# achiever04/face-recognition-platform

Measured on AMD Instinct MI355X. Metric: faces/sec (detect+embed+match) on 1080p @ 100k gallery, higher is better.
Workload: dtype f16; 1 GPU; 32x1080x1920 BGR frames per GPU per step resident in HBM, host results out every step, 2 batches in flight per GPU (one handle = one stream each, used round-robin), forced K=10 faces/frame, 100000-identity fp16 gallery, FRPDet detector fp16 + ArcFace IResNet-100 fp16 (synthetic seeded weights); batch_frames=32, faces_per_frame=10, gallery=100000, streams=1, lanes=2, lane_warmup_steps=20

## Files before the change

### face-recognition-platform_amd/csrc/frp_api.cpp

```cpp
#include <hip/hip_runtime.h>

#include <algorithm>
#include <cmath>
#include <cstdio>
#include <cstdlib>
#include <cstring>
#include <mutex>
#include <string>
#include <vector>

#include "frp.h"
#include "frp_blob.h"
#include "frp_internal.h"
#include "frp_handle.h"

using namespace frp;

#define FRP_WINO_MIN_FACES 128
Switches frp::read_switches() {
    auto set = [](const char* n) { return getenv(n) ? 1 : 0; };
    const char *sm = getenv("FRP_SMALL_M"), *wm = getenv("FRP_WINO_MIN_FACES");
    Switches s{};
    s.small_m = !sm ? 0 : (sm[0] == '0' ? -1 : 1);
    s.wino_min_faces = wm ? atoi(wm) : FRP_WINO_MIN_FACES;
    s.s2 = set("FRP_S2"); s.host_count = set("FRP_HOST_COUNT"); s.match_v1 = set("FRP_MATCH_V1");
    s.no_fused_stem12 = set("FRP_NO_FUSED_STEM12"); s.no_fused_stem = set("FRP_NO_FUSED_STEM");
    s.no_emb_stem = set("FRP_NO_EMB_STEM"); s.no_stem_fuse = set("FRP_NO_STEM_FUSE");
    s.no_wino = set("FRP_NO_WINO"); s.no_kconcat = set("FRP_NO_KCONCAT");
    return s;
}

const ProcessSwitches& frp::process_switches() {
    static const ProcessSwitches s = [] {
        const char* jh = getenv("FRP_JPEG_DEVICE_HUFFMAN");
        const char* js = getenv("FRP_JPEG_SELFSYNC");
        return ProcessSwitches{getenv("FRP_NO_GRAPH") != nullptr, getenv("FRP_C64_ALL") != nullptr, !jh ? 0 : (jh[0] == '0' ? -1 : 1), js && js[0] != '0'};
    }();
    return s;
}

namespace {

float logit_threshold(float t) {
// ... 783 lines not shown
```

### face-recognition-platform_amd/csrc/frp_internal.h

```cpp
#pragma once
#include <hip/hip_runtime.h>
#include <stdint.h>
#include <type_traits>

#define FRP_ACT_NONE 0
#define FRP_ACT_RELU 1
#define FRP_ACT_PRELU 2
#define FRP_FLAG_BORDER_BIAS 1
#define FRP_FLAG_OUT_F32 2
#define FRP_FLAG_RES_UP2 4
#define FRP_FLAG_FLATTEN 8
#define FRP_FLAG_F8 32
#define FRP_FLAG_OUT_FP8 64
#define FRP_CHIP_PIX (112 * 112)
#ifndef FRP_MAX_FACES_CAP
#define FRP_MAX_FACES_CAP 128
#endif

#include "jpeg_host.h"
#include "jpeg_selfsync.h"

namespace frp {

struct Switches {
    int small_m;
    int s2;
    int no_fused_stem12;
    int no_fused_stem;
    int no_emb_stem;
    int no_stem_fuse;
    int wino_min_faces;
    int host_count;
    int match_v1;
    int no_wino;
    int no_kconcat;
};
static_assert(std::has_unique_object_representations_v<Switches>, "run_net keys captured graphs by the bytes of a Switches");
Switches read_switches();

struct ProcessSwitches {
    bool no_graph;
    bool c64_all;
    int jpeg_device_huffman;
    bool jpeg_selfsync;
};
const ProcessSwitches& process_switches();

struct ConvParams {
    const _Float16* x;
    const _Float16* w;
// ... 70 lines not shown
    C64Plan c64;
};
hipError_t conv_derive(ConvParams& p, int* ncu);
ConvRoute conv_pick(const ConvParams& p, int ncu);
hipError_t launch_conv(const ConvParams& p, hipStream_t stream);
hipError_t launch_conv_generic(const ConvParams& p, bool few, hipStream_t stream);
bool conv3x3_rows_eligible(const ConvParams& p);
long conv3x3_lean_default_tiles(const ConvParams& p);
#ifdef FRP_LAB
hipError_t launch_conv3x3_rows(const ConvParams& p, bool few, hipStream_t stream);
#endif
hipError_t launch_conv3x3_lean(const ConvParams& p, bool few, hipStream_t stream);
bool conv3x3_c64_eligible(const ConvParams& p, C64Plan* plan);
bool conv3x3_c64_fuses_stem(int N, int H, int W, int n_cu);
hipError_t launch_conv3x3_c64(const ConvParams& p, const C64Plan& plan, hipStream_t stream);
bool conv3x3_s2_eligible(const ConvParams& p);
hipError_t launch_conv3x3_s2(const ConvParams& p, hipStream_t stream);
int conv3x3_wino_form(const ConvParams& p);
bool conv3x3_wino_shape_ok(int W, int Cin, int ksize, int stride);
bool conv3x3_wino_call_ok(int N, int H, int W, int Cin, int Cout, int ksize, int stride, int n_cu, bool has_res, int dbg);
bool conv3x3_wino_wide_pays(int N, int H, int W, int Cin, int Cout, int n_cu, bool has_res);
#ifdef FRP_LAB
bool conv3x3_wino_lab_shape_ok(int W, int Cin, int ksize, int stride);
#endif
size_t conv3x3_wino_image_bytes(int Cin, int Cout);
hipError_t launch_conv3x3_wino(const ConvParams& p, int form, hipStream_t stream);

hipError_t launch_preprocess(const uint8_t* bgr, int B, int H, int W, long row_stride, long frame_stride,
                             _Float16* out, int Hc, int Wc, int rgb_in, hipStream_t stream);

// ... 272 lines not shown
```

### face-recognition-platform_amd/csrc/kernel_api.cpp

```cpp
#include <hip/hip_runtime.h>

#include <cmath>

#include "frp.h"
#ifdef FRP_LAB
#include "frp_lab.h"
#endif
#include "frp_handle.h"

using namespace frp;

#ifdef FRP_LAB
namespace {
template <typename Launch>
hipError_t time_launches(frp_handle* h, int warm, int iters, Launch launch, float* ms) {
    hipError_t e = hipSuccess;
    for (int i = 0; i < warm && e == hipSuccess; ++i) e = launch();
    if (e == hipSuccess) e = hipEventRecord(h->ev[0], h->stream);
    for (int i = 0; i < iters && e == hipSuccess; ++i) e = launch();
    if (e == hipSuccess) e = hipEventRecord(h->ev[1], h->stream);
    if (e == hipSuccess) e = hipStreamSynchronize(h->stream);
    if (e == hipSuccess) e = hipEventElapsedTime(ms, h->ev[0], h->ev[1]);
    return e;
}
// ... 103 lines not shown
        p.out2 = out2_f8 ? dout2->p : nullptr;
        p.wscale = (const float*)dws->p;
        p.in_scale = in_scale; p.out_scale = out_scale;
        p.N = N; p.H = H; p.W = W; p.Cin = Cin; p.Cout = Cout; p.KS = 3; p.stride = 1; p.act = act;
        p.flags = (flags & (FRP_FLAG_BORDER_BIAS | FRP_FLAG_OUT_FP8)) | FRP_FLAG_F8;
        e = launch_conv(p, h->stream);
    }
    if (e == hipSuccess) e = hipMemcpyAsync(out, dout->p, on * (out8 ? 1 : 2), hipMemcpyDeviceToHost, h->stream);
    if (e == hipSuccess && out2_f8) e = hipMemcpyAsync(out2_f8, dout2->p, on, hipMemcpyDeviceToHost, h->stream);
    hipError_t e2 = hipStreamSynchronize(h->stream);
    if (e != hipSuccess) return fail(h, e == hipErrorInvalidValue ? FRP_ERR_INVALID : FRP_ERR_HIP, std::string("conv2d_f8: ") + hipGetErrorString(e));
    if (e2 != hipSuccess) return fail(h, FRP_ERR_HIP, std::string("conv2d_f8 sync: ") + hipGetErrorString(e2));
    return FRP_OK;
}

int frp_debug_pyramid_merge(frp_handle* h, int32_t n_scales, const int32_t* det_hw, int32_t B, int32_t per_scale, int32_t frame_h,
                            int32_t frame_w, const float* boxes, const float* kps, const float* scores, const int32_t* counts,
                            int32_t max_faces, float nms_iou, float* out_boxes, float* out_kps, float* out_scores, int32_t* out_counts) {
    if (!h) return FRP_ERR_INVALID;
    Guard g(h);
    if (!det_hw || !boxes || !kps || !scores || !counts || !out_boxes || !out_kps || !out_scores || !out_counts)
        return fail(h, FRP_ERR_INVALID, "pyramid_merge: null argument");
    if (n_scales < 1 || n_scales > FRP_PYRAMID_MAX_SCALES || per_scale < 1 || per_scale > FRP_MAX_FACES_CAP ||
        n_scales * per_scale > FRP_PYRAMID_MAX_CAND || max_faces < 1 || max_faces > FRP_MAX_FACES_CAP || B < 1 || B > 1024 || frame_h < 1 ||
        frame_w < 1)
        return fail(h, FRP_ERR_INVALID, "pyramid_merge: 1..4 scales, per_scale and max_faces in 1..128, at most 512 candidates per frame");
    const int S = n_scales, P = per_scale, K = max_faces;
    PyramidMergeParams mp{};
    for (int s = 0; s < S; ++s) {
        mp.det_h[s] = det_hw[2 * s]; mp.det_w[s] = det_hw[2 * s + 1];
// ... 76 lines not shown
        if (with_res) p.out2 = nullptr;
    }
    conv_route_from_abi_flags(flags, p);
    const bool wino_shape = conv3x3_wino_call_ok(N, H, W, Cin, Cout, ksize, stride, h->n_cu, with_res != 0, p.dbg);
    if ((flags & (1 << 16)) && wino_shape) {
        const size_t ib = conv3x3_wino_image_bytes(Cin, Cout);
        if (ensure(h, dwino, ib) == FRP_OK) {
            e = launch_fill_random_f16((_Float16*)dwino->p, (long)(ib / 2), 5u, 1.0f / sqrtf((float)(9 * Cin)), h->stream);
            p.wino_w = (const _Float16*)dwino->p;
        }
    }
    if (stamps_out && ensure(h, dst, 256 * 8 * 8) == FRP_OK) {
        (void)hipMemsetAsync(dst->p, 0, 256 * 8 * 8, h->stream);
        p.stamps = (unsigned long long*)dst->p;
    }
    if (e == hipSuccess) e = time_launches(h, 2, iters, [&] { return launch_conv(p, h->stream); }, &ms);
    if (e == hipSuccess && stamps_out && p.stamps) e = hipMemcpy(stamps_out, p.stamps, 256 * 8 * 8, hipMemcpyDeviceToHost);
    (void)hipStreamSynchronize(h->stream);
    if (e != hipSuccess) return fail(h, FRP_ERR_HIP, std::string("conv_bench: ") + hipGetErrorString(e));
    *ms_avg = ms / iters;
    return FRP_OK;
}

int frp_mfma_peak(frp_handle* h, int32_t waves_per_simd, int32_t iters, float* tflops) {
    if (!h) return FRP_ERR_INVALID;
    Guard g(h);
    const int lds_reads = waves_per_simd >> 4;
    if (lds_reads) waves_per_simd &= 15;
    if (!tflops || iters <= 0 || waves_per_simd < 1 || waves_per_simd > 8 || (lds_reads && (waves_per_simd != 2 || lds_reads < 2 || lds_reads > 4)))
        return fail(h, FRP_ERR_INVALID, "bad arguments");
// ... 39 lines not shown
```

### face-recognition-platform_amd/csrc/net_program.cpp

```cpp
#include "net_program.h"

#include <algorithm>
#include <cmath>
#include <cstdio>
#include <cstring>

#include "frp_handle.h"

namespace frp {

static float fp8_e4m3_value(unsigned char c) {
    const int e = (c >> 3) & 0xF, m = c & 7;
    float v;
    if (e == 15 && m == 7) v = 0.f;
    else if (e == 0) v = std::ldexp((float)m / 8.0f, -6);
    else v = std::ldexp(1.0f + (float)m / 8.0f, e - 7);
    return (c & 0x80) ? -v : v;
}

uint16_t f32_to_f16_bits(float f) {
    uint32_t x;
    memcpy(&x, &f, 4);
    const uint32_t sign = (x >> 16) & 0x8000u;
    x &= 0x7fffffffu;
// ... 234 lines not shown
    if (nb < 0) return;
    const frp_conv_op& b = net.ops[nb];
    const bool plain = !(b.flags & ~FRP_FLAG_BORDER_BIAS) && (b.flags & FRP_FLAG_BORDER_BIAS) && b.out2_buf < 0 && b.res_buf < 0;
    const bool chained = net.kc_src[nb] < 0;
    net.fuse_ok = plain && chained && b.in_buf == a.out_buf && b.out_buf != a.out_buf && b.out_buf != a.in_buf && a.out_buf != a.in_buf &&
                  b.cin == 64 && b.cout == 64 && b.ksize == 3 && b.stride == 1 && b.act == FRP_ACT_PRELU && b.slope_off >= 0;
    net.fuse_even_only = true;
    for (int j = 1; j < (int)net.ops.size(); ++j) {
        const frp_conv_op& o = net.ops[j];
        if (j == nb || (o.in_buf != a.out_buf && o.res_buf != a.out_buf)) continue;
        const bool shortcut = net.kc_skip[j] && o.in_buf == a.out_buf && o.res_buf != a.out_buf && o.ksize == 1 && o.stride == 2;
        if (!shortcut) net.fuse_even_only = false;
    }
}

void analyse_net(Net& net) {
    const int n = (int)net.ops.size();
    net.det_stem = stem_fusable(net);
    net.det_stem12 = stem12_fusable(net);
    net.fc_op = n && (net.ops[n - 1].flags & FRP_FLAG_OUT_F32) ? n - 1 : -1;
    net.next_launch.assign(n, -1);
    for (int i = n - 1, nx = -1; i >= 0; --i) {
        net.next_launch[i] = nx;
        if (!net.kc_skip[i]) nx = i;
    }
    net.emb_stem = net.fuse_ok = net.fuse_even_only = false;
    net.fuse_op = -1;
    if (n) analyse_emb_stem(net);
}

}

int load_program(frp_handle* h, const frp_blob_header& hd, const unsigned char* blob, size_t bytes, const Switches& sw,
                 std::vector<unsigned char>& image) {
    Net &det = h->det, &emb = h->emb;
    det.is_det = true;
    FRPCHK(parse_net(h, blob, bytes, hd.det_ops_offset, hd.n_det_ops, hd.n_det_bufs, hd.det_in_buf, hd.det_in_ch, hd.data_bytes, det));
    FRPCHK(parse_net(h, blob, bytes, hd.emb_ops_offset, hd.n_emb_ops, hd.n_emb_bufs, hd.emb_in_buf, hd.emb_in_ch, hd.data_bytes, emb));
    for (int l = 0; l < 3; ++l)
        if (hd.det_head_buf[l] >= hd.n_det_bufs) return fail(h, FRP_ERR_BLOB, "head buffer id out of range");
    if (hd.emb_out_buf >= hd.n_emb_bufs) return fail(h, FRP_ERR_BLOB, "embedding buffer id out of range");
    image.assign(blob + hd.data_offset, blob + hd.data_offset + hd.data_bytes);
    for (Net* net : {&det, &emb}) {
// ... 1 lines not shown
        net->wino_off.assign(n_ops, -1);
        net->kc_skip.assign(n_ops, 0);
        net->kc_src.assign(n_ops, -1);
        net->kc_w_off.assign(n_ops, -1);
        net->kc_bias_off.assign(n_ops, -1);
        expand_fp8_weights(*net, image);
    }
    if (!sw.no_wino) {
        add_wino_images(emb, FRP_CHIP, [](const frp_conv_op& op, int win) { return conv3x3_wino_shape_ok(win, op.cin, op.ksize, op.stride); }, image);
        add_wino_images(det, 0, [](const frp_conv_op& op, int) { return op.ksize == 3 && op.stride == 1 && !(op.cin & 63) && op.cin >= 128; }, image);
    }
    if (!sw.no_kconcat) {
        plan_kconcat(det, {(int)hd.det_head_buf[0], (int)hd.det_head_buf[1], (int)hd.det_head_buf[2]}, image);
        plan_kconcat(emb, {(int)hd.emb_out_buf}, image);
    }
    analyse_net(det);
    analyse_net(emb);
    return FRP_OK;
}

int plan_net(frp_handle* h, Net& net, int batch, int H, int W, bool skip_input) {
    net.dims.assign(net.n_bufs, TensorDims());
    std::vector<size_t> need(net.n_bufs, 0);
    net.dims[net.in_buf] = {H, W, net.in_ch, false};
    need[net.in_buf] = skip_input ? 0 : (size_t)batch * H * W * net.in_ch * 2;
    for (const frp_conv_op& op : net.ops) {
        if (net.dims[op.in_buf].c == 0) return fail(h, FRP_ERR_BLOB, "program reads an unwritten buffer");
        const TensorDims in = flat_input(net.dims[op.in_buf], op), out = conv_out_dims(in, op);
        if (in.c != op.cin) return fail(h, FRP_ERR_BLOB, "program channel mismatch");
        if (out.h <= 0 || out.w <= 0) return fail(h, FRP_ERR_INVALID, "input too small for the network");
        if (in.f32) return fail(h, FRP_ERR_BLOB, "program reads an fp32 tensor as a conv input");
        const bool op_f8 = (op.flags & FRP_OPFLAG_FP8_MFMA) != 0;
// ... 174 lines not shown
    p.ksplit = ps.n_dev ? -1 : ks;
    p.out = h->splitk_ws.p;
    fc.ksplit = p.ksplit;
    fc.bias = p.bias;
    fc.ktot = op.ksize * op.ksize * op.cin;
}

void charge(const frp_conv_op& op, const TensorDims& out, int batch, PassEffects& fx) {
    const int cin_r = op.real_ch & 0xffff, cout_r = (op.real_ch >> 16) & 0xffff;
    const double fl = 2.0 * batch * out.h * out.w * (double)op.ksize * op.ksize * (cin_r ? cin_r : op.cin) * (cout_r ? cout_r : op.cout);
    fx.flops += fl;
    fx.launches += 1;
    if (op.flags & FRP_OPFLAG_FP8_MFMA) { fx.f8_flops += fl; fx.f8_launches += 1; }
}

int walk(const NetPass& ps, PassEffects& fx) {
    frp_handle* h = ps.h;
    const Net& net = ps.net;
    fx = PassEffects();
    std::vector<TensorDims>& d = fx.dims;
    d.assign(net.n_bufs, TensorDims());
    d[net.in_buf] = {ps.H, ps.W, net.in_ch, false};
    const bool hashing = net.is_det && h->det_hash_on;
    if (hashing) HIPCHK(h, hipMemsetAsync(h->det_hashes.p, 0, 64 * 8, h->stream));
    size_t i = 0;
    FusedStem fused;
    if (ps.stem) FRPCHK(run_det_stems(ps, fx, i));
    else FRPCHK(run_emb_stem(ps, fx, i, fused));
    size_t end = net.ops.size();
    if (net.is_det && h->det_op_limit >= 0) end = std::min(end, (size_t)h->det_op_limit);
    for (; i < end; ++i) {
        const frp_conv_op& op = net.ops[i];
        const TensorDims in = flat_input(d[op.in_buf], op), out = conv_out_dims(in, op);
        if (net.kc_skip[i]) {
            set_out_dims(d, op, out);
            fx.flops += 2.0 * ps.batch * out.h * out.w * (double)op.cin * op.cout;
            continue;
        }
        ConvParams p = conv_params_for(ps, i, in, d, fused);
        if ((int)i == net.fc_op) pick_fc_splitk(ps, op, in, out, p, fx.fc);
        FRPCHK(launched(h, launch_conv(p, h->stream), "launch_conv"));
        set_out_dims(d, op, out);
        if (hashing && i < 64 && !ps.n_dev)
            FRPCHK(launched(h, launch_tensor_hash(net.bufs[op.out_buf].p, (size_t)ps.batch * out.h * out.w * out.c * (out.f32 ? 4 : 2),
                                                  (unsigned long long*)h->det_hashes.p + i, h->stream), "tensor_hash"));
        charge(op, out, ps.batch, fx);
    }
    return FRP_OK;
}

std::string graph_key(const NetPass& ps) {
    char kb[512];
    int len = snprintf(kb, sizeof kb, "%c|%d|%d|%d|%d|%p|%p|", ps.net.is_det ? 'd' : 'e', ps.batch, ps.H, ps.W, (int)ps.allow_wino, (const void*)ps.n_dev,
// ... 95 lines not shown
```

### face-recognition-platform_amd/csrc/net_program.h

```cpp
#pragma once
#include <string>
#include <vector>

#include "frp_blob.h"
#include "frp_internal.h"

struct frp_handle;

namespace frp {

struct DevBuf {
    void* p = nullptr;
    size_t cap = 0;
};

struct TensorDims {
    int h = 0, w = 0, c = 0;
    bool f32 = false;
    bool f8 = false;
};

struct Net {
    std::vector<frp_conv_op> ops;
    int n_bufs = 0;
    int in_buf = 0, in_ch = 0;
    bool is_det = false;
    std::vector<DevBuf> bufs;
    std::vector<TensorDims> dims;
    std::vector<int64_t> wino_off;
    std::vector<int> kc_skip;
    std::vector<int> kc_src;
    std::vector<int64_t> kc_w_off, kc_bias_off;
    bool det_stem = false;
    bool det_stem12 = false;
    bool emb_stem = false;
    int fuse_op = -1;
    bool fuse_ok = false;
    bool fuse_even_only = false;
    int fc_op = -1;
    std::vector<int> next_launch;
};

struct FcSplitK {
    int ksplit = 0, ktot = 0;
    const float* bias = nullptr;
};

struct PassEffects {
    double flops = 0, f8_flops = 0;
    int64_t launches = 0, f8_launches = 0;
    FcSplitK fc;
    std::vector<TensorDims> dims;
};
// ... 24 lines not shown
```

### face-recognition-platform_amd/native.py

```python
from __future__ import annotations

import ctypes as C
import os
import threading
from typing import Optional, Sequence, Tuple

import numpy as np

_HERE = os.path.dirname(os.path.abspath(__file__))
os.environ.setdefault("GPU_MAX_HW_QUEUES", "8")

LIB_PATH = os.environ.get("FRP_LIB") or os.path.join(_HERE, "libfrp.so")

EMB_DIM = 512
CHIP = 112
MAX_FACES_CAP = 128
MAX_TOPK = 64
FLAG_FORCED_K, FLAG_RGB, FLAG_NO_MATCH, FLAG_WITHIN = 1, 2, 4, 8
F32, F16, F64 = 0, 1, 2
JPEG_SUBSAMPLING = {"4:2:0": 420, "4:4:4": 444}
YUV_LAYOUTS = {"NV12": 0, "NV21": 1, "I420": 2, "YV12": 3}
YUV_MATRICES = {"BT601": 0, "BT709": 1, "JFIF": 2}
YUV_DEVICE = 1
QUALITY_TILE_H, QUALITY_TILE_W = 32, 64

ABI_SYMBOLS = [
    "frp_create", "frp_destroy", "frp_last_error", "frp_version", "frp_load_weights",
    "frp_gallery_set", "frp_gallery_set_device", "frp_gallery_reserve", "frp_gallery_commit", "frp_gallery_cancel", "frp_gallery_device_ptr", "frp_gallery_update_row", "frp_gallery_remove_row",
    "frp_jpeg_info_get", "frp_jpeg_coefficients", "frp_upload_jpeg_async", "frp_debug_jpeg_device_batches", "frp_debug_graph_replays",
    "frp_set_jpeg_selfsync", "frp_debug_jpeg_selfsync_batches", "frp_jpeg_selfsync_coefficients",
    "frp_dist_unique_id", "frp_dist_init", "frp_dist_destroy", "frp_gallery_allgather",
    "frp_gallery_size", "frp_gallery_get", "frp_gallery_exact", "frp_gallery_distances", "frp_gallery_get_exact",
    "frp_process_frames", "frp_upload_frames", "frp_process_resident", "frp_fetch_results", "frp_synchronize",
    "frp_host_alloc", "frp_host_free", "frp_upload_frames_async", "frp_swap_frames",
    "frp_upload_yuv", "frp_upload_yuv_async", "frp_get_frames",
    "frp_detect", "frp_detect_resident", "frp_get_det_source", "frp_finish_faces", "frp_process_pyramid", "frp_debug_pyramid_merge", "frp_get_head_map", "frp_debug_det_prefix", "frp_debug_det_hashes", "frp_decode_heads", "frp_align", "frp_debug_align_resident", "frp_embed_aligned", "frp_embed_faces",
    "frp_match", "frp_match_scores", "frp_debug_match_f16", "frp_match_within", "frp_set_within", "frp_fetch_within", "frp_face_quality", "frp_jpeg_encode_headers", "frp_encode_jpeg", "frp_encode_jpeg_coefficients", "frp_conv2d_nhwc", "frp_conv2d_f8", "frp_get_counters", "frp_reset_counters", "frp_set_profile",
]


class FrpConfig(C.Structure):
    _fields_ = [("struct_size", C.c_int32), ("max_batch", C.c_int32), ("max_faces", C.c_int32),
                ("max_h", C.c_int32), ("max_w", C.c_int32), ("profile", C.c_int32), ("reserved", C.c_int32 * 10)]


class FrpCounters(C.Structure):
    _fields_ = [("struct_size", C.c_int32), ("calls", C.c_int32), ("frames", C.c_int64), ("faces", C.c_int64),
                ("ms_h2d", C.c_double), ("ms_preprocess", C.c_double), ("ms_det_conv", C.c_double),
                ("ms_decode", C.c_double), ("ms_align", C.c_double), ("ms_emb_conv", C.c_double),
                ("ms_l2norm", C.c_double), ("ms_match", C.c_double), ("ms_d2h", C.c_double), ("ms_total", C.c_double),
                ("det_conv_flops", C.c_double), ("emb_conv_flops", C.c_double),
                ("det_conv_launches", C.c_int64), ("emb_conv_launches", C.c_int64),
# ... 168 lines not shown
    lib.frp_match_scores.argtypes = [vp, vp, i32, vp, i64]
    if hasattr(lib, "frp_debug_match_f16"):
        lib.frp_debug_match_f16.argtypes = [vp, vp, i32, i32, vp, vp, vp, i64]
    if hasattr(lib, "frp_match_within"):
        lib.frp_match_within.argtypes = [vp, vp, i32, f32, i32, vp, vp, vp]
        lib.frp_set_within.argtypes = [vp, f32, i32]
        lib.frp_fetch_within.argtypes = [vp, i32, i32, i32, vp, vp, vp]
    if hasattr(lib, "frp_face_quality"):
        lib.frp_face_quality.argtypes = [vp, vp, i32, u32, vp]
    if hasattr(lib, "frp_encode_jpeg"):
        lib.frp_jpeg_encode_headers.argtypes = [i32, i32, i32, i32, i32, vp, i64]
        lib.frp_jpeg_encode_headers.restype = i64
        lib.frp_encode_jpeg.argtypes = [vp, vp, i32, i32, i32, i32, u32, vp, i64, vp]
        lib.frp_encode_jpeg_coefficients.argtypes = [vp, vp, i32, i32, i32, u32, vp, i64]
    lib.frp_conv2d_nhwc.argtypes = [vp, vp, i32, i32, i32, i32, vp, i32, i32, i32, vp, vp, vp, i32, i32, i32, i32, vp]
    lib.frp_conv2d_f8.argtypes = [vp, vp, i32, i32, i32, i32, vp, i32, vp, vp, vp, vp, i32, i32, f32, f32, vp, vp]
    if hasattr(lib, "frp_kstep_lab"):
        lib.frp_conv_bench.argtypes = [vp] + [i32] * 11 + [C.POINTER(C.c_float), vp]
        lib.frp_mfma_peak.argtypes = [vp, i32, i32, C.POINTER(C.c_float)]
        lib.frp_kstep_lab.argtypes = [vp, i32, i32, C.POINTER(C.c_float)]
    lib.frp_get_counters.argtypes = [vp, C.POINTER(FrpCounters)]
    lib.frp_reset_counters.argtypes = [vp]
    lib.frp_set_profile.argtypes = [vp, i32]
    _lib = lib
    return lib


def _ptr(a: Optional[np.ndarray]):
    return None if a is None else a.ctypes.data_as(C.c_void_p)

# ... 529 lines not shown
        N, H, W, Cin = x.shape
        Cout, k = w.shape[0], w.shape[1]
        pad = k // 2
        Ho, Wo = (H + 2 * pad - k) // stride + 1, (W + 2 * pad - k) // stride + 1
        out = np.empty((N, Ho, Wo, Cout), dtype=np.float32 if (flags & 2) else np.float16)
        rh = rw = 0
        if res is not None:
            res = np.ascontiguousarray(res, dtype=np.float16)
            rh, rw = res.shape[1], res.shape[2]
        if slope is not None:
            slope = np.ascontiguousarray(slope, dtype=np.float32)
        self._chk(self._lib.frp_conv2d_nhwc(self._h, _ptr(x), N, H, W, Cin, _ptr(w), Cout, k, stride, _ptr(bias), _ptr(slope),
                                            _ptr(res), rh, rw, act, flags, _ptr(out)))
        return out

    def conv2d_f8(self, x8, w8, wscale, bias, act=0, slope=None, res=None, flags=0, in_scale=1.0, out_scale=1.0,
                  out_fp8=False, copy_fp8=False):
        x8 = np.ascontiguousarray(x8, dtype=np.uint8)
        w8 = np.ascontiguousarray(w8, dtype=np.uint8)
        N, H, W, Cin = x8.shape
        Cout = w8.shape[0]
        wscale = np.ascontiguousarray(wscale, dtype=np.float32)
        bias = np.ascontiguousarray(bias, dtype=np.float32)
        if slope is not None:
            slope = np.ascontiguousarray(slope, dtype=np.float32)
        if res is not None:
            res = np.ascontiguousarray(res, dtype=np.float16)
        out = np.empty((N, H, W, Cout), np.uint8 if out_fp8 else np.float16)
        out2 = np.empty((N, H, W, Cout), np.uint8) if copy_fp8 else None
        self._chk(self._lib.frp_conv2d_f8(self._h, _ptr(x8), N, H, W, Cin, _ptr(w8), Cout, _ptr(wscale), _ptr(bias), _ptr(slope),
# ... 42 lines not shown
```

### include/frp.h

```cpp
#ifndef FRP_H
#define FRP_H

#include <stddef.h>
#include <stdint.h>

#ifdef __cplusplus
extern "C" {
#endif

#define FRP_EMB_DIM 512
#define FRP_CHIP 112
#define FRP_KPS 5
#define FRP_MAX_FACES_CAP 128
#define FRP_MAX_TOPK 64

typedef enum frp_status {
    FRP_OK = 0,
    FRP_ERR_INVALID = -1,
    FRP_ERR_HIP = -2,
    FRP_ERR_NO_WEIGHTS = -3,
    FRP_ERR_NO_GALLERY = -4,
    FRP_ERR_BLOB = -5,
    FRP_ERR_OOM = -6
} frp_status;
// ... 149 lines not shown
int frp_face_quality(frp_handle* h, const int32_t* rects, int32_t n, uint32_t flags, int64_t* sums);

#define FRP_JPEG_420 420
#define FRP_JPEG_444 444
int64_t frp_jpeg_encode_headers(int32_t width, int32_t height, int32_t quality, int32_t subsampling, int32_t restart_mcus, uint8_t* out, int64_t cap);
int frp_encode_jpeg(frp_handle* h, const int32_t* rects, int32_t n, int32_t quality, int32_t subsampling, int32_t restart_mcus, uint32_t flags,
                    uint8_t* out, int64_t out_cap, int64_t* offsets);
int frp_encode_jpeg_coefficients(frp_handle* h, const int32_t* rects, int32_t n, int32_t quality, int32_t subsampling, uint32_t flags,
                                 int16_t* coef, int64_t coef_elems);

int frp_conv2d_nhwc(frp_handle* h, const void* x, int32_t N, int32_t H, int32_t W, int32_t Cin,
                    const void* w, int32_t Cout, int32_t ksize, int32_t stride,
                    const float* bias, const float* slope, const void* res, int32_t res_h, int32_t res_w,
                    int32_t act, int32_t flags, void* out);

int frp_conv2d_f8(frp_handle* h, const void* x8, int32_t N, int32_t H, int32_t W, int32_t Cin, const void* w8, int32_t Cout,
                  const float* wscale, const float* bias, const float* slope, const void* res16, int32_t act, int32_t flags,
                  float in_scale, float out_scale, void* out, void* out2_f8);

int frp_get_counters(frp_handle* h, frp_counters* out);
int frp_reset_counters(frp_handle* h);
int frp_set_profile(frp_handle* h, int32_t on);

#ifdef __cplusplus
}
#endif
#endif
```

Measured before the change: 28490 faces/s.

## Fuse consecutive 64-channel 3x3 conv pairs with residual into one block kernel

Adds a kernel that runs two back-to-back 64-channel 3x3 convolutions (a residual basic block) in one launch. The intermediate activation stays in an LDS ring buffer, and the input tile is reused for the residual add. Half the waves compute layer one while the other half compute layer two, pipelined over row groups. A net-analysis pass marks eligible op pairs, and a fill heuristic decides at run time whether to use the fused path. This removes the HBM round trip of the intermediate tensor and one launch per block, at the cost of near-maximal LDS use, halo recompute and a fill-dependent schedule.

```diff
diff --git a/face-recognition-platform_amd/csrc/conv3x3_block64.hip b/face-recognition-platform_amd/csrc/conv3x3_block64.hip
--- /dev/null
+++ b/face-recognition-platform_amd/csrc/conv3x3_block64.hip
@@ -0,0 +1,313 @@
+#include <hip/hip_runtime.h>
+#include <stdint.h>
+#include <stdlib.h>
+#include "frp_internal.h"
+#include "conv_common.h"
+
+namespace frp {
+
+#define B64_PITCH 144
+#define B64_IN_ROW (BLOCK64_IN_W * B64_PITCH)
+#define B64_IN_PIECES 20
+#define B64_IN_GRP (B64_IN_PIECES * 1024)
+#define B64_IN_NGRP 4
+#define B64_MID_ROW (32 * B64_PITCH)
+#define B64_MID_ROWS 16
+#define B64_OFF_MID (B64_IN_NGRP * B64_IN_GRP)
+#define B64_OFF_PAR (B64_OFF_MID + B64_MID_ROWS * B64_MID_ROW + 512)
+#define B64_LDS (B64_OFF_PAR + (9 * 64 + 3 * 64) * 4)
+static_assert(4 * B64_IN_ROW <= B64_IN_GRP && 4 * BLOCK64_IN_W * 9 <= B64_IN_PIECES * 64, "input group");
+static_assert(B64_LDS == BLOCK64_LDS_BYTES && B64_LDS <= 160 * 1024, "LDS budget (frp_internal.h: BLOCK64_LDS_BYTES)");
+#ifndef B64_ABL
+#define B64_ABL 0
+#endif
+
+typedef unsigned b64_u32x4 __attribute__((ext_vector_type(4)));
+
+template <int ACT1, bool BORDER1, int ACT2>
+__global__ __launch_bounds__(512, 2) void conv3x3_block64_kernel(Block64Params p_in) {
+    extern __shared__ __attribute__((aligned(256))) unsigned char smem[];
+    Block64Params p = p_in;
+    int N = p.N;
+    if (p.n_dev) {
+        const int n = *p.n_dev;
+        N = n < 0 ? 0 : (n > p.N ? p.N : n);
+    }
+    const int t = threadIdx.x;
+    const int lane = t & 63;
+    const int wave = __builtin_amdgcn_readfirstlane(t >> 6);
+    const int layer = wave >> 2, wl = wave & 3, wc = wl & 1, wp = wl >> 1;
+    const int fr = lane & 31, fh = lane >> 5;
+    const int per_img = p.strips * p.segs;
+    const int n_items = N * per_img;
+    const int H = p.H, W = p.W;
+
+    const unsigned io_bytes = (unsigned)((long)p.N * H * W * 128);
+    const __amdgpu_buffer_rsrc_t xrsrc = __builtin_amdgcn_make_buffer_rsrc((void*)p.x, 0, io_bytes, 0x00020000);
+    const __amdgpu_buffer_rsrc_t orsrc = __builtin_amdgcn_make_buffer_rsrc(p.out, 0, io_bytes, 0x00020000);
+
+    float* lds_bias1 = reinterpret_cast<float*>(smem + B64_OFF_PAR);
+    float* lds_slope1 = lds_bias1 + 9 * 64;
+    float* lds_bias2 = lds_slope1 + 64;
+    float* lds_slope2 = lds_bias2 + 64;
+    for (int i = t; i < 9 * 64; i += 512) lds_bias1[i] = (BORDER1 || i < 64) ? p.bias1[i] : 0.f;
+    if (t < 64) {
+        lds_slope1[t] = (ACT1 == FRP_ACT_PRELU && p.slope1) ? p.slope1[t] : 0.f;
+        lds_bias2[t] = p.bias2[t];
+        lds_slope2[t] = (ACT2 == FRP_ACT_PRELU && p.slope2) ? p.slope2[t] : 0.f;
+    }
+
+    half8 A[36];
+    {
+        const _Float16* wrow = (layer ? p.w2 : p.w1) + (long)(wc * 32 + fr) * 576 + 8 * fh;
+#pragma unroll
+        for (int s = 0; s < 36; ++s) A[s] = *reinterpret_cast<const half8*>(wrow + (s >> 2) * 64 + (s & 3) * 16);
+    }
+    __syncthreads();
+
+    int lane_e = lane;
+    const int lbase = fr * B64_PITCH + fh * 16;
+    floatx16 acc[2];
+
+    for (int item = blockIdx.x; item < n_items; item += gridDim.x) {
+        const Block64Item wi = block64_item(item, p.strips, p.segs, p.seg_rows, H);
+        const int n = wi.n, ys = wi.ys, ye = wi.ye, x0 = wi.x0, K = wi.K;
+
+        retire_lds_reads();
+        __builtin_amdgcn_s_barrier();
+
+        auto multiply = [&](const auto& rp) __attribute__((always_inline)) {
+#pragma unroll
+            for (int b = 0; b < 2; ++b)
+#pragma unroll
+                for (int e = 0; e < 16; ++e) acc[b][e] = 0.f;
+            half8 bf[3][2];
+            auto rd = [&](int s, int S) {
+                const int tap = s >> 2, kk = s & 3;
+#pragma unroll
+                for (int b = 0; b < 2; ++b)
+                    bf[S][b] = *reinterpret_cast<const half8*>(rp[b + tap / 3] + (tap % 3) * B64_PITCH + kk * 32);
+            };
+            rd(0, 0);
+            rd(1, 1);
+#pragma unroll
+            for (int s = 0; s < 36; ++s) {
+                if (s + 2 < 36) rd(s + 2, (s + 2) % 3);
+                if (!(B64_ABL & 4)) {
+#pragma unroll
+                    for (int b = 0; b < 2; ++b) acc[b] = __builtin_amdgcn_mfma_f32_32x32x16_f16(A[s], bf[s % 3][b], acc[b], 0, 0, 0);
+                } else {
+                    asm volatile("" ::"v"(bf[s % 3][0]), "v"(bf[s % 3][1]));
+                }
+                __builtin_amdgcn_sched_barrier(0);
+            }
+        };
+
+        if (layer == 0) {
+            auto issue_group = [&](int g) {
+                if (B64_ABL & 2) return;
+                const int gy = ys - 6 + 4 * g;
+                unsigned char* dst = smem + (g & 3) * B64_IN_GRP;
+#pragma unroll
+                for (int j = 0; j < 5; ++j) {
+                    const int piece = wl + 4 * j;
+                    const int sl = piece * 64 + lane_e;
+                    const int R = (sl * 7282) >> 16, chunk = sl - 9 * R;
+                    const int py = (R * 241) >> 13, px = R - py * BLOCK64_IN_W;
+                    const int y = gy + py, x = x0 - 2 + px;
+                    const bool ok = R < 4 * BLOCK64_IN_W && chunk < 8 && (unsigned)y < (unsigned)H && (unsigned)x < (unsigned)W;
+                    dma16(xrsrc, dst + piece * 1024, ok ? (unsigned)(((n * H + y) * W + x) * 128 + chunk * 16) : CONV_OOB);
+                }
+            };
+            issue_group(1);
+            issue_group(2);
+            for (int k = 0; k <= K; ++k) {
+                wait_vmcnt<0>();
+                retire_lds_reads();
+                __builtin_amdgcn_s_barrier();
+                if (k == K) break;
+                asm volatile("" : "+v"(lane_e));
+                if (k + 3 <= K + 1) issue_group(k + 3);
+                const int ib = 4 * (k + 1) + 2 * wp;
+                const unsigned char* rp[4];
+#pragma unroll
+                for (int j = 0; j < 4; ++j) {
+                    const int i = ib + j;
+                    rp[j] = smem + (((i >> 2) & 3) * B64_IN_GRP + (i & 3) * B64_IN_ROW) + lbase;
+                }
+                multiply(rp);
+#pragma unroll
+                for (int b = 0; b < 2; ++b) {
+                    const int my = ys - 1 + 4 * k + 2 * wp + b, mx = x0 - 1 + fr;
+                    const bool inimg = (unsigned)my < (unsigned)H && (unsigned)mx < (unsigned)W;
+                    int cls = 0;
+                    if (BORDER1) cls = ((my == 0) ? 0 : (my == H - 1) ? 2 : 1) * 3 + ((mx == 0) ? 0 : (mx == W - 1) ? 2 : 1);
+                    if (!inimg) cls = 0;
+                    union { half4 h; unsigned u[2]; } pk[4];
+#pragma unroll
+                    for (int g = 0; g < 4; ++g) {
+                        const int cl = wc * 32 + 8 * g + 4 * fh;
+                        const floatx4 b4 = *reinterpret_cast<const floatx4*>(lds_bias1 + cls * 64 + cl);
+                        floatx4 v;
+#pragma unroll
+                        for (int e = 0; e < 4; ++e) v[e] = acc[b][4 * g + e] + b4[e];
+                        if (ACT1 == FRP_ACT_RELU) {
+#pragma unroll
+                            for (int e = 0; e < 4; ++e) v[e] = fmaxf(v[e], 0.f);
+                        } else if (ACT1 == FRP_ACT_PRELU) {
+                            const floatx4 s4 = *reinterpret_cast<const floatx4*>(lds_slope1 + cl);
+#pragma unroll
+                            for (int e = 0; e < 4; ++e) v[e] = v[e] > 0.f ? v[e] : v[e] * s4[e];
+                        }
+#pragma unroll
+                        for (int e = 0; e < 4; ++e) pk[g].h[e] = (_Float16)v[e];
+                    }
+                    const int ms = (6 + 4 * k + 2 * wp + b) & (B64_MID_ROWS - 1);
+                    unsigned char* mrow = smem + B64_OFF_MID + ms * B64_MID_ROW + lbase + wc * 64;
+#pragma unroll
+                    for (int q = 0; q < 2; ++q) {
+                        swap_halves(pk[2 * q].u[0], pk[2 * q + 1].u[0]);
+                        swap_halves(pk[2 * q].u[1], pk[2 * q + 1].u[1]);
+                        b64_u32x4 o = {pk[2 * q].u[0], pk[2 * q].u[1], pk[2 * q + 1].u[0], pk[2 * q + 1].u[1]};
+                        if (!inimg) o = b64_u32x4{0u, 0u, 0u, 0u};
+                        *reinterpret_cast<b64_u32x4*>(mrow + q * 32) = o;
+                    }
+                }
+            }
+        } else {
+            for (int k = 0; k <= K; ++k) {
+                retire_lds_reads();
+                __builtin_amdgcn_s_barrier();
+                if (k == 0) continue;
+                const int ib = 4 * k + 2 * wp;
+                const unsigned char* rp[4];
+#pragma unroll
+                for (int j = 0; j < 4; ++j) rp[j] = smem + B64_OFF_MID + ((ib + j) & (B64_MID_ROWS - 1)) * B64_MID_ROW + lbase;
+                multiply(rp);
+                b64_u32x4 rr[2][2];
+                unsigned ooff[2];
+#pragma unroll
+                for (int b = 0; b < 2; ++b) {
+                    const int oy = ys - 6 + 4 * k + 2 * wp + b, ox = x0 + fr;
+                    const bool ok = oy >= ys && oy < ye && fr < BLOCK64_STRIP_W && ox < W;
+                    ooff[b] = ok ? (unsigned)(((n * H + oy) * W + ox) * 128 + wc * 64 + fh * 16) : CONV_OOB;
+                    const int i = ib + b;
+                    const unsigned char* xr = smem + (((i >> 2) & 3) * B64_IN_GRP + (i & 3) * B64_IN_ROW) + lbase + 2 * B64_PITCH + wc * 64;
+#pragma unroll
+                    for (int q = 0; q < 2; ++q) rr[b][q] = *reinterpret_cast<const b64_u32x4*>(xr + q * 32);
+                }
+#pragma unroll
+                for (int b = 0; b < 2; ++b) {
+                    half4 r4[4];
+#pragma unroll
+                    for (int q = 0; q < 2; ++q) {
+                        b64_u32x4 v = rr[b][q];
+                        unsigned x_ = v.x, y_ = v.y, z_ = v.z, w_ = v.w;
+                        swap_halves(x_, z_);
+                        swap_halves(y_, w_);
+                        union { unsigned u[2]; half4 h; } lo, hi;
+                        lo.u[0] = x_; lo.u[1] = y_; hi.u[0] = z_; hi.u[1] = w_;
+                        r4[2 * q] = lo.h;
+                        r4[2 * q + 1] = hi.h;
+                    }
+                    union { half4 h; unsigned u[2]; } pk[4];
+#pragma unroll
+                    for (int g = 0; g < 4; ++g) {
+                        const int cl = wc * 32 + 8 * g + 4 * fh;
+                        const floatx4 b4 = *reinterpret_cast<const floatx4*>(lds_bias2 + cl);
+                        floatx4 v;
+#pragma unroll
+                        for (int e = 0; e < 4; ++e) v[e] = acc[b][4 * g + e] + b4[e];
+#pragma unroll
+                        for (int e = 0; e < 4; ++e) v[e] += (float)r4[g][e];
+                        if (ACT2 == FRP_ACT_RELU) {
+#pragma unroll
+                            for (int e = 0; e < 4; ++e) v[e] = fmaxf(v[e], 0.f);
+                        } else if (ACT2 == FRP_ACT_PRELU) {
+                            const floatx4 s4 = *reinterpret_cast<const floatx4*>(lds_slope2 + cl);
+#pragma unroll
+                            for (int e = 0; e < 4; ++e) v[e] = v[e] > 0.f ? v[e] : v[e] * s4[e];
+                        }
+#pragma unroll
+                        for (int e = 0; e < 4; ++e) pk[g].h[e] = (_Float16)v[e];
+                    }
+#pragma unroll
+                    for (int q = 0; q < 2; ++q) {
+                        swap_halves(pk[2 * q].u[0], pk[2 * q + 1].u[0]);
+                        swap_halves(pk[2 * q].u[1], pk[2 * q + 1].u[1]);
+                        const b64_u32x4 o = {pk[2 * q].u[0], pk[2 * q].u[1], pk[2 * q + 1].u[0], pk[2 * q + 1].u[1]};
+                        if (B64_ABL & 1) asm volatile("" ::"v"(o)); else
+                        __builtin_amdgcn_raw_buffer_store_b128(o, orsrc, ooff[b] + 32 * q, 0, 0);
+                    }
+                }
+            }
+        }
+    }
+    wait_vmcnt<0>();
+}
+
+int conv3x3_block64_variant(int act1, int flags1, bool slope1, int act2, int flags2) {
+    if (flags2 != 0 || (flags1 & ~FRP_FLAG_BORDER_BIAS)) return 0;
+    const bool border = (flags1 & FRP_FLAG_BORDER_BIAS) != 0;
+    if (act1 == FRP_ACT_RELU && !border && act2 == FRP_ACT_RELU) return 1;
+    if (act1 == FRP_ACT_PRELU && border && slope1 && act2 == FRP_ACT_NONE) return 2;
+    return 0;
+}
+
+bool conv3x3_block64_plan(int N, int H, int W, int n_cu, Block64Plan* g) {
+    *g = Block64Plan{};
+    if (N <= 0 || H <= 0 || W <= 0 || (long)N * H * W * 128 >= 0x7f000000L) return false;
+    const int ncu = n_cu > 0 ? n_cu : 256;
+    const int strips = (W + BLOCK64_STRIP_W - 1) / BLOCK64_STRIP_W;
+    long best = -1;
+    for (int want : {1, 2, 4, 8}) {
+        const int rows = ((H + want - 1) / want + 3) / 4 * 4;
+        if (want > 1 && rows < 8) break;
+        const int segs = (H + rows - 1) / rows;
+        const int steps = ((rows < H ? rows : H) + 2 + 3) / 4 + 1;
+        const long items = (long)N * strips * segs, rounds = (items + ncu - 1) / ncu;
+        if (items > 0x7fffffffL) continue;
+        const long cost = rounds * steps;
+        if (best < 0 || cost < best) {
+            best = cost;
+            g->strips = strips; g->segs = segs; g->seg_rows = rows; g->steps = steps; g->items = items;
+            g->grid = (int)(items < ncu ? items : ncu);
+            g->fill = (double)N * H * W / ((double)rounds * ncu * steps * (4.0 * BLOCK64_STRIP_W));
+        }
+    }
+    g->lds = B64_LDS;
+    return best >= 0;
+}
+
+bool conv3x3_block64_pays(const Block64Plan& g) {
+    return g.items > 0 && g.fill >= BLOCK64_MIN_FILL;
+}
+
+template <int ACT1, bool BORDER1, int ACT2>
+static hipError_t launch_block64_as(const Block64Params& p, int grid, hipStream_t stream) {
+    static int attr_done[64] = {};
+    int dev = 0, ncu = 0;
+    hipError_t e = conv_device(&dev, &ncu);
+    if (e != hipSuccess) return e;
+    if (!attr_done[dev]) {
+        e = hipFuncSetAttribute(reinterpret_cast<const void*>(conv3x3_block64_kernel<ACT1, BORDER1, ACT2>), hipFuncAttributeMaxDynamicSharedMemorySize, B64_LDS);
+        if (e != hipSuccess) return e;
+        attr_done[dev] = 1;
+    }
+    hipLaunchKernelGGL((conv3x3_block64_kernel<ACT1, BORDER1, ACT2>), dim3(grid), dim3(512), B64_LDS, stream, p);
+    return hipGetLastError();
+}
+
+hipError_t launch_conv3x3_block64(const Block64Params& p0, hipStream_t stream) {
+    Block64Params p = p0;
+    Block64Plan g;
+    if (!p.x || !p.w1 || !p.bias1 || !p.w2 || !p.bias2 || !p.out || p.x == p.out) return hipErrorInvalidValue;
+    const int variant = conv3x3_block64_variant(p.act1, p.flags1, p.slope1 != nullptr, p.act2, 0);
+    if (!variant || ((p.flags1 & FRP_FLAG_BORDER_BIAS) && (p.H < 2 || p.W < 2))) return hipErrorInvalidValue;
+    if (!conv3x3_block64_plan(p.N, p.H, p.W, p.n_cu, &g)) return hipErrorInvalidValue;
+    p.strips = g.strips; p.segs = g.segs; p.seg_rows = g.seg_rows;
+    return variant == 1 ? launch_block64_as<FRP_ACT_RELU, false, FRP_ACT_RELU>(p, g.grid, stream)
+                        : launch_block64_as<FRP_ACT_PRELU, true, FRP_ACT_NONE>(p, g.grid, stream);
+}
+
+}
diff --git a/face-recognition-platform_amd/csrc/frp_api.cpp b/face-recognition-platform_amd/csrc/frp_api.cpp
--- a/face-recognition-platform_amd/csrc/frp_api.cpp
+++ b/face-recognition-platform_amd/csrc/frp_api.cpp
@@ -27,6 +27,7 @@
     s.no_fused_stem12 = set("FRP_NO_FUSED_STEM12"); s.no_fused_stem = set("FRP_NO_FUSED_STEM");
     s.no_emb_stem = set("FRP_NO_EMB_STEM"); s.no_stem_fuse = set("FRP_NO_STEM_FUSE");
     s.no_wino = set("FRP_NO_WINO"); s.no_kconcat = set("FRP_NO_KCONCAT");
+    s.no_block_fuse = set("FRP_NO_BLOCK_FUSE"); s.block_fuse_all = set("FRP_BLOCK_FUSE_ALL");
     return s;
 }
 
diff --git a/face-recognition-platform_amd/csrc/frp_internal.h b/face-recognition-platform_amd/csrc/frp_internal.h
--- a/face-recognition-platform_amd/csrc/frp_internal.h
+++ b/face-recognition-platform_amd/csrc/frp_internal.h
@@ -34,6 +34,8 @@
     int match_v1;
     int no_wino;
     int no_kconcat;
+    int no_block_fuse;
+    int block_fuse_all;
 };
 static_assert(std::has_unique_object_representations_v<Switches>, "run_net keys captured graphs by the bytes of a Switches");
 Switches read_switches();
@@ -134,6 +136,52 @@
 bool conv3x3_c64_eligible(const ConvParams& p, C64Plan* plan);
 bool conv3x3_c64_fuses_stem(int N, int H, int W, int n_cu);
 hipError_t launch_conv3x3_c64(const ConvParams& p, const C64Plan& plan, hipStream_t stream);
+#define BLOCK64_STRIP_W 30
+#define BLOCK64_IN_W 34
+#define BLOCK64_LDS_BYTES 159232
+#define BLOCK64_MIN_FILL 0.70
+struct Block64Params {
+    const _Float16* x;
+    const _Float16* w1;
+    const float* bias1;
+    const float* slope1;
+    const _Float16* w2;
+    const float* bias2;
+    const float* slope2;
+    void* out;
+    const int32_t* n_dev;
+    int N, H, W;
+    int act1, flags1, act2;
+    int n_cu;
+    int strips, segs, seg_rows;
+};
+struct Block64Plan {
+    int strips, segs, seg_rows;
+    int steps;
+    long items;
+    int grid, lds;
+    double fill;
+};
+struct Block64Item { int n, ys, ye, x0, K; };
+__host__ __device__ inline Block64Item block64_item(int item, int strips, int segs, int seg_rows, int H) {
+    Block64Item it;
+    const int per_img = strips * segs;
+    it.n = item / per_img;
+    const int r = item - it.n * per_img, seg = r / strips;
+    it.ys = seg * seg_rows;
+    it.ye = it.ys + seg_rows < H ? it.ys + seg_rows : H;
+    it.x0 = (r - seg * strips) * BLOCK64_STRIP_W;
+    it.K = (it.ye - it.ys + 2 + 3) >> 2;
+    return it;
+}
+#define BLOCK64_HALO_UP 2
+#define BLOCK64_HALO_DOWN 7
+__host__ __device__ inline int block64_first_in_row(const Block64Item& it) { return it.ys - 6 + 4; }
+__host__ __device__ inline int block64_last_in_row(const Block64Item& it) { return it.ys - 6 + 4 * (it.K + 1) + 3; }
+int conv3x3_block64_variant(int act1, int flags1, bool slope1, int act2, int flags2);
+bool conv3x3_block64_plan(int N, int H, int W, int n_cu, Block64Plan* plan);
+bool conv3x3_block64_pays(const Block64Plan& plan);
+hipError_t launch_conv3x3_block64(const Block64Params& p, hipStream_t stream);
 bool conv3x3_s2_eligible(const ConvParams& p);
 hipError_t launch_conv3x3_s2(const ConvParams& p, hipStream_t stream);
 int conv3x3_wino_form(const ConvParams& p);
diff --git a/face-recognition-platform_amd/csrc/kernel_api.cpp b/face-recognition-platform_amd/csrc/kernel_api.cpp
--- a/face-recognition-platform_amd/csrc/kernel_api.cpp
+++ b/face-recognition-platform_amd/csrc/kernel_api.cpp
@@ -141,6 +141,59 @@
     return FRP_OK;
 }
 
+int frp_conv_block64(frp_handle* h, const void* x, int32_t N, int32_t H, int32_t W, const void* w1, const float* bias1, const float* slope1,
+                     int32_t act1, int32_t flags1, const void* w2, const float* bias2, const float* slope2, int32_t act2, void* out) {
+    if (!h) return FRP_ERR_INVALID;
+    Guard g(h);
+    if (!x || !w1 || !bias1 || !w2 || !bias2 || !out || N <= 0 || H <= 0 || W <= 0) return fail(h, FRP_ERR_INVALID, "bad block arguments");
+    if (!conv3x3_block64_variant(act1, flags1, slope1 != nullptr, act2, 0)) return fail(h, FRP_ERR_INVALID, "block epilogues not covered by the fused kernel");
+    Block64Plan plan;
+    if (!conv3x3_block64_plan(N, H, W, h->n_cu, &plan) || ((flags1 & FRP_FLAG_BORDER_BIAS) && (H < 2 || W < 2)))
+        return fail(h, FRP_ERR_INVALID, "block shape out of the fused kernel's reach");
+    const size_t tb = (size_t)N * H * W * 128, wb = (size_t)64 * 576 * 2, guard = 4096;
+    const size_t b1 = (size_t)64 * 4 * ((flags1 & FRP_FLAG_BORDER_BIAS) ? 9 : 1);
+    ScopedBuf dx, dw1, dw2, db1, db2, ds1, ds2, dout;
+    FRPCHK(ensure(h, dx, tb + 2 * guard));
+    FRPCHK(ensure(h, dout, tb + 2 * guard));
+    FRPCHK(ensure(h, dw1, wb));
+    FRPCHK(ensure(h, dw2, wb));
+    FRPCHK(ensure(h, db1, b1));
+    FRPCHK(ensure(h, db2, 256));
+    if (slope1) FRPCHK(ensure(h, ds1, 256));
+    if (slope2) FRPCHK(ensure(h, ds2, 256));
+    std::vector<uint16_t> nan(guard, 0x7e00u), back(guard);
+    char *gx = (char*)dx->p, *go = (char*)dout->p;
+    hipError_t e = hipMemcpyAsync(gx, nan.data(), guard, hipMemcpyHostToDevice, h->stream);
+    if (e == hipSuccess) e = hipMemcpyAsync(gx + guard + tb, nan.data(), guard, hipMemcpyHostToDevice, h->stream);
+    if (e == hipSuccess) e = hipMemcpyAsync(go, nan.data(), guard, hipMemcpyHostToDevice, h->stream);
+    if (e == hipSuccess) e = hipMemcpyAsync(go + guard + tb, nan.data(), guard, hipMemcpyHostToDevice, h->stream);
+    if (e == hipSuccess) e = hipMemsetAsync(go + guard, 0x7e, tb, h->stream);
+    if (e == hipSuccess) e = hipMemcpyAsync(gx + guard, x, tb, hipMemcpyHostToDevice, h->stream);
+    if (e == hipSuccess) e = hipMemcpyAsync(dw1->p, w1, wb, hipMemcpyHostToDevice, h->stream);
+    if (e == hipSuccess) e = hipMemcpyAsync(dw2->p, w2, wb, hipMemcpyHostToDevice, h->stream);
+    if (e == hipSuccess) e = hipMemcpyAsync(db1->p, bias1, b1, hipMemcpyHostToDevice, h->stream);
+    if (e == hipSuccess) e = hipMemcpyAsync(db2->p, bias2, 256, hipMemcpyHostToDevice, h->stream);
+    if (e == hipSuccess && slope1) e = hipMemcpyAsync(ds1->p, slope1, 256, hipMemcpyHostToDevice, h->stream);
+    if (e == hipSuccess && slope2) e = hipMemcpyAsync(ds2->p, slope2, 256, hipMemcpyHostToDevice, h->stream);
+    if (e == hipSuccess) {
+        Block64Params p{};
+        p.x = (const _Float16*)(gx + guard); p.out = go + guard;
+        p.w1 = (const _Float16*)dw1->p; p.bias1 = (const float*)db1->p; p.slope1 = slope1 ? (const float*)ds1->p : nullptr;
+        p.w2 = (const _Float16*)dw2->p; p.bias2 = (const float*)db2->p; p.slope2 = slope2 ? (const float*)ds2->p : nullptr;
+        p.N = N; p.H = H; p.W = W; p.act1 = act1; p.flags1 = flags1; p.act2 = act2;
+        p.n_cu = h->n_cu;
+        e = launch_conv3x3_block64(p, h->stream);
+    }
+    if (e == hipSuccess) e = hipMemcpyAsync(out, go + guard, tb, hipMemcpyDeviceToHost, h->stream);
+    if (e == hipSuccess) e = hipMemcpyAsync(back.data(), go, guard, hipMemcpyDeviceToHost, h->stream);
+    if (e == hipSuccess) e = hipMemcpyAsync((char*)back.data() + guard, go + guard + tb, guard, hipMemcpyDeviceToHost, h->stream);
+    hipError_t e2 = hipStreamSynchronize(h->stream);
+    if (e != hipSuccess) return fail(h, e == hipErrorInvalidValue ? FRP_ERR_INVALID : FRP_ERR_HIP, std::string("conv_block64: ") + hipGetErrorString(e));
+    if (e2 != hipSuccess) return fail(h, FRP_ERR_HIP, std::string("conv_block64 sync: ") + hipGetErrorString(e2));
+    if (back != nan) return fail(h, FRP_ERR_HIP, "conv_block64: the launch wrote outside its output tensor");
+    return FRP_OK;
+}
+
 int frp_debug_pyramid_merge(frp_handle* h, int32_t n_scales, const int32_t* det_hw, int32_t B, int32_t per_scale, int32_t frame_h,
                             int32_t frame_w, const float* boxes, const float* kps, const float* scores, const int32_t* counts,
                             int32_t max_faces, float nms_iou, float* out_boxes, float* out_kps, float* out_scores, int32_t* out_counts) {
@@ -247,6 +300,14 @@
         (void)hipMemsetAsync(dst->p, 0, 256 * 8 * 8, h->stream);
         p.stamps = (unsigned long long*)dst->p;
     }
+    if (flags & (1 << 23)) {
+        Block64Params bp{};
+        bp.x = p.x; bp.out = p.out; bp.w1 = bp.w2 = p.w; bp.bias1 = bp.bias2 = p.bias; bp.slope1 = p.slope;
+        bp.N = N; bp.H = H; bp.W = W; bp.act1 = act; bp.flags1 = flags & FRP_FLAG_BORDER_BIAS; bp.act2 = act == FRP_ACT_RELU ? FRP_ACT_RELU : FRP_ACT_NONE;
+        bp.n_cu = h->n_cu;
+        if (Cin != 64 || Cout != 64 || ksize != 3 || stride != 1) e = hipErrorInvalidValue;
+        if (e == hipSuccess) e = time_launches(h, 2, iters, [&] { return launch_conv3x3_block64(bp, h->stream); }, &ms);
+    } else
     if (e == hipSuccess) e = time_launches(h, 2, iters, [&] { return launch_conv(p, h->stream); }, &ms);
     if (e == hipSuccess && stamps_out && p.stamps) e = hipMemcpy(stamps_out, p.stamps, 256 * 8 * 8, hipMemcpyDeviceToHost);
     (void)hipStreamSynchronize(h->stream);
diff --git a/face-recognition-platform_amd/csrc/net_program.cpp b/face-recognition-platform_amd/csrc/net_program.cpp
--- a/face-recognition-platform_amd/csrc/net_program.cpp
+++ b/face-recognition-platform_amd/csrc/net_program.cpp
@@ -272,7 +272,31 @@
     }
 }
 
-void analyse_net(Net& net) {
+void analyse_block64(Net& net, const std::vector<int>& read_outside) {
+    const int n = (int)net.ops.size();
+    net.block64.assign(n, 0);
+    for (int i = 0; i + 1 < n; ++i) {
+        const frp_conv_op &a = net.ops[i], &b = net.ops[i + 1];
+        auto c64 = [](const frp_conv_op& o) { return o.ksize == 3 && o.stride == 1 && o.cin == 64 && o.cout == 64 && o.out2_buf < 0; };
+        if (!c64(a) || !c64(b) || net.kc_skip[i] || net.kc_skip[i + 1] || net.kc_src[i] >= 0 || net.kc_src[i + 1] >= 0) continue;
+        if (a.res_buf >= 0 || b.in_buf != a.out_buf || b.res_buf != a.in_buf || b.out_buf == a.in_buf || b.out_buf == a.out_buf) continue;
+        if (a.in_buf == net.in_buf && net.in_ch != 64) continue;
+        if (!conv3x3_block64_variant(a.act, a.flags, a.slope_off >= 0, b.act, b.flags)) continue;
+        if (net.fuse_ok && i == net.fuse_op) continue;
+        bool ok = true;
+        for (int q = i + 2; q < n && ok; ++q) {
+            const frp_conv_op& o = net.ops[q];
+            if (o.in_buf == a.out_buf || o.res_buf == a.out_buf) ok = false;
+            if (o.out_buf == a.out_buf || o.out2_buf == a.out_buf) break;
+        }
+        for (int r : read_outside) ok &= r != a.out_buf;
+        if (!ok) continue;
+        net.block64[i] = 1;
+        ++i;
+    }
+}
+
+void analyse_net(Net& net, const std::vector<int>& read_outside) {
     const int n = (int)net.ops.size();
     net.det_stem = stem_fusable(net);
     net.det_stem12 = stem12_fusable(net);
@@ -285,6 +309,7 @@
     net.emb_stem = net.fuse_ok = net.fuse_even_only = false;
     net.fuse_op = -1;
     if (n) analyse_emb_stem(net);
+    analyse_block64(net, read_outside);
 }
 
 }
@@ -316,8 +341,8 @@
         plan_kconcat(det, {(int)hd.det_head_buf[0], (int)hd.det_head_buf[1], (int)hd.det_head_buf[2]}, image);
         plan_kconcat(emb, {(int)hd.emb_out_buf}, image);
     }
-    analyse_net(det);
-    analyse_net(emb);
+    analyse_net(det, {(int)hd.det_head_buf[0], (int)hd.det_head_buf[1], (int)hd.det_head_buf[2]});
+    analyse_net(emb, {(int)hd.emb_out_buf});
     return FRP_OK;
 }
 
@@ -522,6 +547,14 @@
     if (op.flags & FRP_OPFLAG_FP8_MFMA) { fx.f8_flops += fl; fx.f8_launches += 1; }
 }
 
+bool block64_fuses(const NetPass& ps, const TensorDims& in) {
+    if (ps.sw.no_block_fuse || ps.sw.small_m > 0) return false;
+    Block64Plan plan;
+    if (!conv3x3_block64_plan(ps.batch, in.h, in.w, ps.h->n_cu, &plan)) return false;
+    if ((in.h < 2 || in.w < 2)) return false;
+    return ps.sw.block_fuse_all || conv3x3_block64_pays(plan);
+}
+
 int walk(const NetPass& ps, PassEffects& fx) {
     frp_handle* h = ps.h;
     const Net& net = ps.net;
@@ -545,6 +578,29 @@
             fx.flops += 2.0 * ps.batch * out.h * out.w * (double)op.cin * op.cout;
             continue;
         }
+        if (net.block64[i] && i + 1 < end && !hashing && block64_fuses(ps, in)) {
+            const frp_conv_op& op2 = net.ops[i + 1];
+            const char* wbase = ps.weights();
+            Block64Params bp{};
+            bp.x = (const _Float16*)net.bufs[op.in_buf].p;
+            bp.out = net.bufs[op2.out_buf].p;
+            bp.w1 = (const _Float16*)(wbase + op.w_off); bp.bias1 = (const float*)(wbase + op.bias_off);
+            bp.slope1 = op.slope_off >= 0 ? (const float*)(wbase + op.slope_off) : nullptr;
+            bp.w2 = (const _Float16*)(wbase + op2.w_off); bp.bias2 = (const float*)(wbase + op2.bias_off);
+            bp.slope2 = op2.slope_off >= 0 ? (const float*)(wbase + op2.slope_off) : nullptr;
+            bp.n_dev = ps.n_dev;
+            bp.N = ps.batch; bp.H = in.h; bp.W = in.w;
+            bp.act1 = op.act; bp.flags1 = op.flags & FRP_FLAG_BORDER_BIAS; bp.act2 = op2.act;
+            bp.n_cu = h->n_cu;
+            FRPCHK(launched(h, launch_conv3x3_block64(bp, h->stream), "launch_conv3x3_block64"));
+            set_out_dims(d, op, out);
+            set_out_dims(d, op2, out);
+            charge(op, out, ps.batch, fx);
+            charge(op2, out, ps.batch, fx);
+            fx.launches -= 1;
+            ++i;
+            continue;
+        }
         ConvParams p = conv_params_for(ps, i, in, d, fused);
         if ((int)i == net.fc_op) pick_fc_splitk(ps, op, in, out, p, fx.fc);
         FRPCHK(launched(h, launch_conv(p, h->stream), "launch_conv"));
diff --git a/face-recognition-platform_amd/csrc/net_program.h b/face-recognition-platform_amd/csrc/net_program.h
--- a/face-recognition-platform_amd/csrc/net_program.h
+++ b/face-recognition-platform_amd/csrc/net_program.h
@@ -37,6 +37,7 @@
     int fuse_op = -1;
     bool fuse_ok = false;
     bool fuse_even_only = false;
+    std::vector<char> block64;
     int fc_op = -1;
     std::vector<int> next_launch;
 };
diff --git a/face-recognition-platform_amd/native.py b/face-recognition-platform_amd/native.py
--- a/face-recognition-platform_amd/native.py
+++ b/face-recognition-platform_amd/native.py
@@ -35,7 +35,7 @@
     "frp_host_alloc", "frp_host_free", "frp_upload_frames_async", "frp_swap_frames",
     "frp_upload_yuv", "frp_upload_yuv_async", "frp_get_frames",
     "frp_detect", "frp_detect_resident", "frp_get_det_source", "frp_finish_faces", "frp_process_pyramid", "frp_debug_pyramid_merge", "frp_get_head_map", "frp_debug_det_prefix", "frp_debug_det_hashes", "frp_decode_heads", "frp_align", "frp_debug_align_resident", "frp_embed_aligned", "frp_embed_faces",
-    "frp_match", "frp_match_scores", "frp_debug_match_f16", "frp_match_within", "frp_set_within", "frp_fetch_within", "frp_face_quality", "frp_jpeg_encode_headers", "frp_encode_jpeg", "frp_encode_jpeg_coefficients", "frp_conv2d_nhwc", "frp_conv2d_f8", "frp_get_counters", "frp_reset_counters", "frp_set_profile",
+    "frp_match", "frp_match_scores", "frp_debug_match_f16", "frp_match_within", "frp_set_within", "frp_fetch_within", "frp_face_quality", "frp_jpeg_encode_headers", "frp_encode_jpeg", "frp_encode_jpeg_coefficients", "frp_conv2d_nhwc", "frp_conv_block64", "frp_conv2d_f8", "frp_get_counters", "frp_reset_counters", "frp_set_profile",
 ]
 
 
@@ -234,6 +234,8 @@
         lib.frp_encode_jpeg.argtypes = [vp, vp, i32, i32, i32, i32, u32, vp, i64, vp]
         lib.frp_encode_jpeg_coefficients.argtypes = [vp, vp, i32, i32, i32, u32, vp, i64]
     lib.frp_conv2d_nhwc.argtypes = [vp, vp, i32, i32, i32, i32, vp, i32, i32, i32, vp, vp, vp, i32, i32, i32, i32, vp]
+    if hasattr(lib, "frp_conv_block64"):
+        lib.frp_conv_block64.argtypes = [vp, vp, i32, i32, i32, vp, vp, vp, i32, i32, vp, vp, vp, i32, vp]
     lib.frp_conv2d_f8.argtypes = [vp, vp, i32, i32, i32, i32, vp, i32, vp, vp, vp, vp, i32, i32, f32, f32, vp, vp]
     if hasattr(lib, "frp_kstep_lab"):
         lib.frp_conv_bench.argtypes = [vp] + [i32] * 11 + [C.POINTER(C.c_float), vp]
@@ -793,6 +795,26 @@
                                             _ptr(res), rh, rw, act, flags, _ptr(out)))
         return out
 
+    def conv_block64(self, x, w1, bias1, w2, bias2, act1=1, act2=1, slope1=None, slope2=None, flags1=0):
+        x = np.ascontiguousarray(x, dtype=np.float16)
+        w1 = np.ascontiguousarray(w1, dtype=np.float16)
+        w2 = np.ascontiguousarray(w2, dtype=np.float16)
+        bias1 = np.ascontiguousarray(bias1, dtype=np.float32)
+        bias2 = np.ascontiguousarray(bias2, dtype=np.float32)
+        if x.ndim != 4 or x.shape[3] != 64 or w1.shape != (64, 3, 3, 64) or w2.shape != (64, 3, 3, 64):
+            raise ValueError("conv_block64: x [N,H,W,64], w1 / w2 [64,3,3,64]")
+        if bias1.size != (576 if flags1 & 1 else 64) or bias2.size != 64:
+            raise ValueError("conv_block64: bias1 [64] ([9,64] with border classes), bias2 [64]")
+        if slope1 is not None:
+            slope1 = np.ascontiguousarray(slope1, dtype=np.float32)
+        if slope2 is not None:
+            slope2 = np.ascontiguousarray(slope2, dtype=np.float32)
+        N, H, W, _ = x.shape
+        out = np.empty_like(x)
+        self._chk(self._lib.frp_conv_block64(self._h, _ptr(x), N, H, W, _ptr(w1), _ptr(bias1), _ptr(slope1), act1, flags1,
+                                             _ptr(w2), _ptr(bias2), _ptr(slope2), act2, _ptr(out)))
+        return out
+
     def conv2d_f8(self, x8, w8, wscale, bias, act=0, slope=None, res=None, flags=0, in_scale=1.0, out_scale=1.0,
                   out_fp8=False, copy_fp8=False):
         x8 = np.ascontiguousarray(x8, dtype=np.uint8)
diff --git a/include/frp.h b/include/frp.h
--- a/include/frp.h
+++ b/include/frp.h
@@ -187,6 +187,10 @@
                     const float* bias, const float* slope, const void* res, int32_t res_h, int32_t res_w,
                     int32_t act, int32_t flags, void* out);
 
+int frp_conv_block64(frp_handle* h, const void* x, int32_t N, int32_t H, int32_t W, const void* w1, const float* bias1,
+                     const float* slope1, int32_t act1, int32_t flags1, const void* w2, const float* bias2, const float* slope2,
+                     int32_t act2, void* out);
+
 int frp_conv2d_f8(frp_handle* h, const void* x8, int32_t N, int32_t H, int32_t W, int32_t Cin, const void* w8, int32_t Cout,
                   const float* wscale, const float* bias, const float* slope, const void* res16, int32_t act, int32_t flags,
                   float in_scale, float out_scale, void* out, void* out2_f8);
```

Result: faster. 28960 faces/s, median of 6 (+1.6%).
